# LiuZhu-CV/PAIF

Hardware: AMD Instinct MI355X
Metric: fused image-pairs/sec at 480x640 bs=8 per GPU (fusion-net forward) (higher is better)
Workload: dtype f16 (IEEE fp16 maps and conv weights, one fp16 MFMA per product, f32 accumulate; stems, guided filter and the last map fp32)

## Files before the change

paif_amd/csrc/conv_dma.hip:

```cpp
#include <stdint.h>
#include <stdlib.h>

#include <type_traits>

#include "conv_dma.h"
#include "conv_rows.h"

namespace paif_conv_dma {
namespace {

using namespace paif_rows;
constexpr int TW = 32, TH = 8;
#ifndef CD_PF
#define CD_PF 4
#endif
#ifndef CD_ST_AUX
#define CD_ST_AUX 2
#endif
#ifndef CD_EPI_SWAP
#define CD_EPI_SWAP 1
#endif
#ifndef CD_EPI_LINES
#define CD_EPI_LINES 1
#endif
#ifndef CD_EXP
#define CD_EXP 0
#endif
constexpr int PARK_WAVE = 2 * 32 * 32 * 4;
template <int DIL>
struct Geo {
  static constexpr int TWH = TW + 2 * DIL, THH = TH + 2 * DIL;
  static constexpr int NPIX = TWH * THH;
  static constexpr int DPW = (NPIX * 4 + 255) / 256;
  static constexpr int SLOT = 4 * DPW * 1024;
  static constexpr int PF = DIL == 1 ? CD_PF : 3;
  static constexpr int NSLOT = PF + 1;
  static constexpr int ROWB = TWH * 64;
  static constexpr int PARK_OFF = NSLOT * SLOT;
  static constexpr int lds_bytes(bool parked) { return PARK_OFF + (parked ? 4 * PARK_WAVE : 0); }
  static_assert(lds_bytes(true) <= 160 * 1024, "ring + transposition buffers exceed LDS");
  static_assert(4 * DPW * 64 >= NPIX * 4, "DMA instructions do not cover the halo tile");
  static __device__ __forceinline__ int base_row(int w) { return DIL == 1 ? 2 * w : (w >> 1) * 4 + (w & 1); }
};
constexpr int NSTORE = 4;
constexpr int VMCAP = 63;

#define CD_VMWAIT(n) ROWS_VMWAIT((n) > VMCAP ? VMCAP : (n))

template <int NSRC, int NRES, int PF, int DPW>
struct Sched {
  static constexpr int RL = 4 * NRES;
  static constexpr int smod(int x) { return ((x % NSRC) + NSRC) % NSRC; }
  static constexpr int R_STAGE = smod(1 - PF);
  static constexpr int D = (R_STAGE + PF - 1 - NSRC) / NSRC;
  static constexpr int U = D + (R_STAGE == 0 ? 2 : 1);
  static_assert(PF >= 2 && D >= 0 && U <= 4, "prefetch distance out of the range the tile loop lists");
  static constexpr int n1 = DPW * (PF - 1);
};

template <int NSRC, int NRES, int F, bool CP = false, int DIL = 1, int IA = 0>
__global__ __launch_bounds__(256, 1) void conv3x3_h16_dma(Args a, int ntiles, int tilesX, int tilesY) {
  typedef Geo<DIL> G;
  constexpr int TWH = G::TWH, NPIX = G::NPIX, DPW = G::DPW, SLOT = G::SLOT, PF = G::PF, NSLOT = G::NSLOT, ROWB = G::ROWB, PARK_OFF = G::PARK_OFF;
  typedef Sched<NSRC, NRES, PF, DPW> SC;
  constexpr bool SW = CD_EPI_SWAP && !CP && !(NRES == 3 && (NSRC == 3 || DIL == 2));
  constexpr int U = SW ? (SC::U + 1) & ~1 : SC::U, D = SC::D;
  constexpr int NACC = SW ? 2 : 1;
  __shared__ __attribute__((aligned(16))) unsigned char smem[G::lds_bytes(!SW)];
  asm volatile("" ::"v"((unsigned)(uintptr_t)(__attribute__((address_space(3))) unsigned char*)smem) : "memory");

  const int tid = threadIdx.x, l = tid & 63;
  const int w = __builtin_amdgcn_readfirstlane(tid >> 6);
  const int p = l & 31, hh = l >> 5;
  const int wb = G::base_row(w);

  const int xcd = blockIdx.x & 7, wg = blockIdx.x >> 3, nwg = gridDim.x >> 3;
  const int tpx = (ntiles + 7) >> 3;
  const int t_beg = xcd * tpx, t_end = min(ntiles, t_beg + tpx);
  const int cnt = t_beg + wg < t_end ? (t_end - t_beg - wg + nwg - 1) / nwg : 0;
  if (cnt == 0) return;
  const int H = a.H, W = a.W;
  auto pack_tile = [&](int k) -> unsigned {
    const int pos = wg + min(k, cnt - 1) * nwg;
    int t = a.reverse ? t_end - 1 - pos : t_beg + pos;
    const int tx = t % tilesX;
    t /= tilesX;
    const int ty = t % tilesY;
    return ((unsigned)(t / tilesY) << 22) | ((unsigned)ty << 11) | (unsigned)tx;
  };
  const unsigned tab0 = pack_tile(l), tab1 = pack_tile(l + 64);
  auto tile_of = [&](int k, int& b, int& y0, int& x0) -> bool {
    const bool ok = k >= 0 && k < cnt;
    const int kk = ok ? k : 0;
    const unsigned lo = __builtin_amdgcn_readlane(tab0, kk & 63), hi = __builtin_amdgcn_readlane(tab1, kk & 63);
    const unsigned pk = kk < 64 ? lo : hi;
    b = pk >> 22; y0 = ((pk >> 11) & 2047) * TH; x0 = (pk & 2047) * TW;
    return ok;
  };

  const int map_bytes = a.B * H * W * 64;
  __amdgpu_buffer_rsrc_t rs_src[NSRC];
#pragma unroll
  for (int s = 0; s < NSRC; ++s) rs_src[s] = __builtin_amdgcn_make_buffer_rsrc(const_cast<void*>(a.src[s]), 0, map_bytes, RSRC_W3);
  __amdgpu_buffer_rsrc_t rs_res[NRES > 0 ? NRES : 1];
#pragma unroll
  for (int r = 0; r < NRES; ++r) rs_res[r] = __builtin_amdgcn_make_buffer_rsrc(const_cast<void*>(a.res[r]), 0, map_bytes, RSRC_W3);
  const int opitch = a.cout * 2;
  const __amdgpu_buffer_rsrc_t rs_out = __builtin_amdgcn_make_buffer_rsrc(a.out, 0, a.B * H * W * opitch, RSRC_W3);
  const __amdgpu_buffer_rsrc_t rs_null = __builtin_amdgcn_make_buffer_rsrc(a.out, 0, 0, RSRC_W3);
  const __amdgpu_buffer_rsrc_t rs_cp = __builtin_amdgcn_make_buffer_rsrc(CP ? (void*)a.cpool : a.out, 0, CP ? a.B * H * W * 16 - 8 : 0, RSRC_W3);

  u32x4 bw[NSRC][9][2];
  {
    const __amdgpu_buffer_rsrc_t rs_w = __builtin_amdgcn_make_buffer_rsrc(const_cast<void*>(a.wpk), 0, NSRC * 9 * 2 * 2 * 1024, RSRC_W3);
#pragma unroll
    for (int s = 0; s < NSRC; ++s)
#pragma unroll
      for (int tap = 0; tap < 9; ++tap)
#pragma unroll
        for (int ks = 0; ks < 2; ++ks)
          bw[s][tap][ks] = __builtin_amdgcn_raw_buffer_load_b128(rs_w, (unsigned)l * 16u, (((s * 9 + tap) * 2 + ks) * 2) * 1024, 0);
  }
  constexpr int NEC = SW ? 16 : 8;
  float esc[NEC], esh[NEC];
#pragma unroll
  for (int j = 0; j < NEC; ++j) {
    const int c = SW ? ROWS_ACC_CHANNEL(j, hh) : 8 * (l & 3) + j;
    esc[j] = ((a.scale && c < a.cout) ? a.scale[c] : 1.f) * a.alpha;
    esh[j] = ((a.shift && c < a.cout) ? a.shift[c] : 0.f) * a.alpha;
  }
  const float e_slope = a.act == 1 ? *a.prelu : (a.act == 2 ? 0.f : 1.f);

  int d_rel[DPW];
  int d_rc[DPW];
#pragma unroll
  for (int i = 0; i < DPW; ++i) {
    const int n = (w * DPW + i) * 64 + l;
    const int pi = n >> 2;
    const int r = pi / TWH, c = pi - r * TWH;
    d_rel[i] = (r * W + c) * 64 + (((n & 3) ^ ((c >> 2) & 3)) * 16);
    d_rc[i] = pi < NPIX ? (r | (c << 8)) : -1;
  }
  unsigned d_voff[DPW];
  auto target = [&](int k) {
    int b, y0, x0;
    const bool ok = tile_of(k, b, y0, x0);
    const int org = ((b * H + y0 - DIL) * W + x0 - DIL) * 64;
#pragma unroll
    for (int i = 0; i < DPW; ++i) {
      const int gy = y0 - DIL + (d_rc[i] & 0xff), gx = x0 - DIL + (d_rc[i] >> 8);
      const bool in = !(CD_EXP & 4) && ok && d_rc[i] >= 0 && (unsigned)gy < (unsigned)H && (unsigned)gx < (unsigned)W;
      d_voff[i] = in ? (unsigned)(org + d_rel[i]) : OOB;
    }
  };
  unsigned a_rd[3][2];
#pragma unroll
  for (int dx = 0; dx < 3; ++dx)
#pragma unroll
    for (int ks = 0; ks < 2; ++ks) {
      const int c = p + dx * DIL;
      a_rd[dx][ks] = (unsigned)(wb * ROWB + c * 64 + (((2 * ks + hh) ^ ((c >> 2) & 3)) * 16));
    }
  const unsigned a_pw = PARK_OFF + w * PARK_WAVE + (4 * hh * 32 + p) * 4;
  const unsigned a_pr = PARK_OFF + w * PARK_WAVE + (l >> 2) * 128 + (l & 3) * 32;
  const unsigned e_lane = (unsigned)l * 16u;
  const unsigned o_lane = 8 * (l & 3) < a.cout ? (unsigned)((l >> 2) * opitch + (l & 3) * 16) : OOB;
  const unsigned e_lane_sw = (unsigned)(p * 64 + hh * 16);
  const unsigned o_lane_sw = (unsigned)(p * opitch + hh * 16);
  const unsigned o_lane_ln = ((l >> 4) & 1) * 16 < a.cout ? (unsigned)((l & 15) * opitch + ((l >> 4) & 1) * 32 + (l >> 5) * 16) : OOB;

  u32x4 rr[U][NRES > 0 ? NRES : 1][4];
  auto issue_res = [&](auto settag, int k) {
    constexpr int SET = decltype(settag)::value;
    int b, y0, x0;
    const bool ok = tile_of(k, b, y0, x0);
#pragma unroll
    for (int it = 0; it < 4; ++it) {
      const int y = y0 + wb + (it >> 1) * DIL, x = SW ? x0 + p : x0 + (it & 1) * 16 + (l >> 2);
      const bool in = ok && y < H && x < W;
      const unsigned soff = SW ? (unsigned)(((b * H + y) * W + x0) * 64 + (it & 1) * 32) : (unsigned)(((b * H + y) * W + x0 + (it & 1) * 16) * 64);
      const unsigned voff = in ? (SW ? e_lane_sw : e_lane) : OOB;
#pragma unroll
      for (int r = 0; r < NRES; ++r) rr[SET][r][it] = __builtin_amdgcn_raw_buffer_load_b128(rs_res[r], voff, soff, 0);
    }
  };

  auto relu_frag = [](u32x4& f) {
    typedef short s16x8 __attribute__((ext_vector_type(8)));
    const s16x8 z = {0, 0, 0, 0, 0, 0, 0, 0};
    f = __builtin_bit_cast(u32x4, __builtin_elementwise_max(__builtin_bit_cast(s16x8, f), z));
  };
  f32x16 acc[NACC][2];
  if constexpr (SW) {
#pragma unroll
    for (int r = 0; r < 16; ++r) acc[1][0][r] = acc[1][1][r] = 0.f;
  }
  u32x4 t[4][2];
#pragma unroll
  for (int it = 0; it < 4; ++it) t[it][0] = t[it][1] = u32x4{0, 0, 0, 0};
  float ev[8];
  u32x4 oq[2];
  float pmx = 0.f, psm = 0.f;
  int cur = NSLOT - PF;

  auto epi_park = [&](auto mtag, auto settag, bool pok, int pb, int py0, int px0) {
    constexpr int M = decltype(mtag)::value, SETP = decltype(settag)::value;
    constexpr int it = M / 9, j = M % 9;
    if constexpr (j < 8) {
      const unsigned raw = j < 4 ? t[it][0][j & 3] : t[it][1][j & 3];
      float v = __builtin_fmaf(__uint_as_float(raw), esc[j], esh[j]);
      v = __builtin_fmaf(e_slope, fminf(v, 0.f), fmaxf(v, 0.f));
#pragma unroll
      for (int r = 0; r < NRES; ++r) {
        const unsigned u = rr[SETP][r][it][j >> 1];
        if constexpr (F == 2) v += (float)__builtin_bit_cast(paif::f16x2_t, u)[j & 1];
        else v += __uint_as_float((j & 1) ? (u & 0xffff0000u) : (u << 16));
      }
      ev[j] = v;
      if constexpr (CP) {
        pmx = j == 0 ? v : fmaxf(pmx, v);
        psm = j == 0 ? v : psm + v;
      }
    } else {
      const uint2 o0 = paif::f32_to_h4<F>(make_float4(ev[0], ev[1], ev[2], ev[3]));
      const uint2 o1 = paif::f32_to_h4<F>(make_float4(ev[4], ev[5], ev[6], ev[7]));
      const int y = py0 + wb + (it >> 1) * DIL, x = px0 + (it & 1) * 16 + (l >> 2);
      const unsigned soff = (unsigned)(((pb * H + y) * W + px0 + (it & 1) * 16) * opitch);
      u32x4 od = {o0.x, o0.y, o1.x, o1.y};
      __builtin_amdgcn_raw_buffer_store_b128(od, rs_out, (!(CD_EXP & 1) && pok && y < H && x < W) ? o_lane : OOB, soff, CD_ST_AUX);
      asm volatile("s_nop 2" : "+v"(od));
      if constexpr (CP) {
        float mx = pmx, sm = psm;
        mx = fmaxf(mx, paif::dpp_f<0xB1>(mx)); sm += paif::dpp_f<0xB1>(sm);
        mx = fmaxf(mx, paif::dpp_f<0x4E>(mx)); sm += paif::dpp_f<0x4E>(sm);
        typedef float f32x2v __attribute__((ext_vector_type(2)));
        const f32x2v pv = {mx, sm * (1.0f / 32.0f)};
        const unsigned poff = (unsigned)(((pb * H + y) * W + px0 + (it & 1) * 16) * 16);
        __builtin_amdgcn_raw_buffer_store_b64(__builtin_bit_cast(unsigned __attribute__((ext_vector_type(2))), pv), rs_cp,
                                              (pok && y < H && x < W && (l & 3) == 0) ? (unsigned)((l >> 2) * 16) : OOB, poff, 0);
      }
    }
  };
  auto epi_swap = [&](auto mtag, auto settag, auto aptag, bool pok, int pb, int py0, int px0) {
    constexpr int M = decltype(mtag)::value, SETP = decltype(settag)::value, AP = decltype(aptag)::value;
    constexpr int row = M / 18, q = M % 18;
    if constexpr (q < 16) {
      constexpr int it = 2 * row + (q >> 3), j = q & 7;
      if constexpr (j == 0) {
#pragma unroll
        for (int r = 0; r < NRES; ++r) rr[SETP][r][it] = swap_unpack(rr[SETP][r][it]);
      }
      float v = __builtin_fmaf(acc[AP][row][q], esc[q], esh[q]);
      v = __builtin_fmaf(e_slope, fminf(v, 0.f), fmaxf(v, 0.f));
#pragma unroll
      for (int r = 0; r < NRES; ++r) {
        const unsigned u = rr[SETP][r][it][j >> 1];
        if constexpr (F == 2) v += (float)__builtin_bit_cast(paif::f16x2_t, u)[j & 1];
        else v += __uint_as_float((j & 1) ? (u & 0xffff0000u) : (u << 16));
      }
      if constexpr ((j & 1) == 0) ev[0] = v;
      else oq[q >> 3][j >> 1] = f32_to_h2<F>(ev[0], v);
    } else if constexpr (q == 16) {
      oq[0] = swap_unpack(oq[0]);
      oq[1] = swap_unpack(oq[1]);
      if constexpr (CD_EPI_LINES) line_swap(oq[0], oq[1]);
    } else {
      const int y = py0 + wb + row * DIL;
      const unsigned soff = (unsigned)(((pb * H + y) * W + px0) * opitch);
      const bool ok = !(CD_EXP & 1) && pok && y < H;
      if constexpr (CD_EPI_LINES) {
        const int x = px0 + (l & 15);
        __builtin_amdgcn_raw_buffer_store_b128(oq[0], rs_out, (ok && x < W) ? o_lane_ln : OOB, soff, CD_ST_AUX);
        __builtin_amdgcn_raw_buffer_store_b128(oq[1], rs_out, (ok && x + 16 < W) ? o_lane_ln : OOB, soff + (unsigned)(16 * opitch), CD_ST_AUX);
      } else {
        const int x = px0 + p;
        __builtin_amdgcn_raw_buffer_store_b128(oq[0], rs_out, (ok && x < W) ? o_lane_sw : OOB, soff, CD_ST_AUX);
        __builtin_amdgcn_raw_buffer_store_b128(oq[1], rs_out, (ok && x < W && a.cout > 16) ? o_lane_sw + 32u : OOB, soff, CD_ST_AUX);
      }
      asm volatile("s_nop 2" : "+v"(oq[0]), "+v"(oq[1]));
    }
  };
  auto epi = [&](auto mtag, auto settag, auto aptag, bool pok, int pb, int py0, int px0) {
    if constexpr (SW) epi_swap(mtag, settag, aptag, pok, pb, py0, px0);
    else epi_park(mtag, settag, pok, pb, py0, px0);
  };

  auto stage = [&](auto ktag, auto stag, auto virt, int k) {
    constexpr int K = decltype(ktag)::value, S = decltype(stag)::value;
    constexpr bool VIRT = decltype(virt)::value;
    constexpr int SETP = (K + U - 1) % U;
    constexpr int AC = SW ? K & 1 : 0, AP = SW ? AC ^ 1 : 0;
    const unsigned sb = (unsigned)cur * SLOT;
    const int fill = cur == 0 ? NSLOT - 1 : cur - 1;
    u32x4 A[2][4];
    unsigned ad[3][2];
    if constexpr (!VIRT) {
      CD_VMWAIT(SC::n1);
      asm volatile("s_barrier" ::: "memory");
#pragma unroll
      for (int dx = 0; dx < 3; ++dx)
#pragma unroll
        for (int ks = 0; ks < 2; ++ks) ad[dx][ks] = a_rd[dx][ks] + sb;
      if constexpr (S == 0 && !SW) {
#pragma unroll
        for (int it = 0; it < 4; ++it) {
          ROWS_RD128(t[it][0], a_pr, it * 2048);
          ROWS_RD128(t[it][1], a_pr, it * 2048 + 16);
        }
      }
#pragma unroll
      for (int r = 0; r < 4; ++r) ROWS_RD128(A[0][r], ad[0][0], r * DIL * ROWB);
    }
    if constexpr (NRES > 0 && S == SC::R_STAGE) issue_res(std::integral_constant<int, (K + D) % U>{}, k + D);
    asm volatile("" ::: "memory");
    if constexpr ((S + PF) % NSRC == 0) target(k + (S + PF) / NSRC);
#pragma unroll
    for (int i = 0; i < DPW; ++i) dma16<0>(rs_src[(S + PF) % NSRC], d_voff[i], (unsigned)(fill * SLOT + (w * DPW + i) * 1024));
    if constexpr (VIRT) {
      if constexpr (S == 0) {
#pragma unroll
        for (int it = 0; it < NSTORE; ++it) __builtin_amdgcn_raw_buffer_store_b128(u32x4{0, 0, 0, 0}, rs_null, 0, 0, 0);
      }
    } else {
      int pb = 0, py0 = 0, px0 = 0;
      bool pok = false;
      if constexpr (S == 0) pok = tile_of(k - 1, pb, py0, px0);
      auto mma = [&](auto gitag, auto dytag, auto jtag) {
        constexpr int gi = decltype(gitag)::value, dy = decltype(dytag)::value, j = decltype(jtag)::value;
        constexpr int ks = gi / 3, dx = gi % 3;
        if constexpr (!((CD_EXP & 2) && (dy > 0 || j > 0))) {
          const u32x4 pv = A[gi & 1][j + dy], wv = bw[S][dy * 3 + dx][ks];
          const u32x4 av = SW ? wv : pv, bv = SW ? pv : wv;
          if constexpr (S == 0 && gi == 0 && dy == 0) {
            const f32x16 z = {0.f, 0.f, 0.f, 0.f, 0.f, 0.f, 0.f, 0.f, 0.f, 0.f, 0.f, 0.f, 0.f, 0.f, 0.f, 0.f};
            acc[AC][j] = paif::mfma16<F>(av, bv, z);
          } else {
            acc[AC][j] = paif::mfma16<F>(av, bv, acc[AC][j]);
          }
        }
        if constexpr (S == 0)
          epi(std::integral_constant<int, gi * 6 + dy * 2 + j>{}, std::integral_constant<int, SETP>{}, std::integral_constant<int, AP>{}, pok, pb, py0, px0);
        if constexpr (IA == 2) {
          constexpr int call = dy * 2 + j;
          if constexpr (call == 0) relu_frag(A[gi & 1][1]);
          if constexpr (call == 2) relu_frag(A[gi & 1][2]);
          if constexpr (call == 4) relu_frag(A[gi & 1][3]);
        }
        __builtin_amdgcn_sched_barrier(0);
      };
      auto group = [&](auto gitag) {
        constexpr int gi = decltype(gitag)::value;
        if constexpr (gi + 1 < 6) {
          constexpr int ks1 = (gi + 1) / 3, dx1 = (gi + 1) % 3;
#pragma unroll
          for (int r = 0; r < 4; ++r) ROWS_RD128(A[(gi + 1) & 1][r], ad[dx1][ks1], r * DIL * ROWB);
        }
        if constexpr (S == 0 && gi == 0 && !SW) {
          asm volatile("s_waitcnt lgkmcnt(4)"
                       : "+v"(A[0][0]), "+v"(A[0][1]), "+v"(A[0][2]), "+v"(A[0][3]), "+v"(t[0][0]), "+v"(t[0][1]), "+v"(t[1][0]), "+v"(t[1][1]),
                         "+v"(t[2][0]), "+v"(t[2][1]), "+v"(t[3][0]), "+v"(t[3][1])::"memory");
        } else if constexpr (gi + 1 < 6) {
          asm volatile("s_waitcnt lgkmcnt(4)" : "+v"(A[gi & 1][0]), "+v"(A[gi & 1][1]), "+v"(A[gi & 1][2]), "+v"(A[gi & 1][3])::"memory");
        } else {
          asm volatile("s_waitcnt lgkmcnt(0)" : "+v"(A[gi & 1][0]), "+v"(A[gi & 1][1]), "+v"(A[gi & 1][2]), "+v"(A[gi & 1][3])::"memory");
        }
        if constexpr (IA == 2) relu_frag(A[gi & 1][0]);
        __builtin_amdgcn_sched_barrier(0);
        typedef std::integral_constant<int, 0> I0;
        typedef std::integral_constant<int, 1> I1;
        typedef std::integral_constant<int, 2> I2;
        mma(gitag, I0{}, I0{}); mma(gitag, I0{}, I1{});
        mma(gitag, I1{}, I0{}); mma(gitag, I1{}, I1{});
        mma(gitag, I2{}, I0{}); mma(gitag, I2{}, I1{});
      };
      group(std::integral_constant<int, 0>{});
      group(std::integral_constant<int, 1>{});
      group(std::integral_constant<int, 2>{});
      group(std::integral_constant<int, 3>{});
      group(std::integral_constant<int, 4>{});
      group(std::integral_constant<int, 5>{});
      if constexpr (S == NSRC - 1 && !SW) {
        asm volatile("s_nop 15\n\ts_nop 7" ::: "memory");
#pragma unroll
        for (int j = 0; j < 2; ++j)
#pragma unroll
          for (int r = 0; r < 16; ++r) {
            const float v = acc[0][j][r];
            ROWS_WR32(a_pw, v, (j * 32 + (r & 3) + 8 * (r >> 2)) * 128);
          }
      }
    }
    cur = cur == NSLOT - 1 ? 0 : cur + 1;
  };
  auto drain = [&](auto ktag, int k) {
    constexpr int K = decltype(ktag)::value;
    if constexpr (!SW) {
#pragma unroll
      for (int it = 0; it < 4; ++it) {
        ROWS_RD128(t[it][0], a_pr, it * 2048);
        ROWS_RD128(t[it][1], a_pr, it * 2048 + 16);
      }
      asm volatile("s_waitcnt lgkmcnt(0)"
                   : "+v"(t[0][0]), "+v"(t[0][1]), "+v"(t[1][0]), "+v"(t[1][1]), "+v"(t[2][0]), "+v"(t[2][1]), "+v"(t[3][0]), "+v"(t[3][1])::"memory");
    }
    int pb, py0, px0;
    const bool pok = tile_of(k, pb, py0, px0);
#define CD_M(m) epi(std::integral_constant<int, m>{}, std::integral_constant<int, K>{}, std::integral_constant<int, (SW ? K & 1 : 0)>{}, pok, pb, py0, px0);
    CD_M(0) CD_M(1) CD_M(2) CD_M(3) CD_M(4) CD_M(5) CD_M(6) CD_M(7) CD_M(8) CD_M(9) CD_M(10) CD_M(11)
    CD_M(12) CD_M(13) CD_M(14) CD_M(15) CD_M(16) CD_M(17) CD_M(18) CD_M(19) CD_M(20) CD_M(21) CD_M(22) CD_M(23)
    CD_M(24) CD_M(25) CD_M(26) CD_M(27) CD_M(28) CD_M(29) CD_M(30) CD_M(31) CD_M(32) CD_M(33) CD_M(34) CD_M(35)
#undef CD_M
  };

  auto vstage = [&](auto jtag) {
    constexpr int J = decltype(jtag)::value;
    constexpr int T = (J - (NSRC - 1)) / NSRC;
    constexpr int S = J - T * NSRC;
    constexpr int K = ((T % U) + U) % U;
    stage(std::integral_constant<int, K>{}, std::integral_constant<int, S>{}, std::true_type{}, T);
  };
  static_assert(PF >= 1 && PF <= 4, "the prologue lists up to 4 virtual stages");
  if constexpr (PF >= 4) vstage(std::integral_constant<int, -4>{});
  if constexpr (PF >= 3) vstage(std::integral_constant<int, -3>{});
  if constexpr (PF >= 2) vstage(std::integral_constant<int, -2>{});
  vstage(std::integral_constant<int, -1>{});

  auto tile_step = [&](auto ktag, int k) {
    stage(ktag, std::integral_constant<int, 0>{}, std::false_type{}, k);
    if constexpr (NSRC > 1) stage(ktag, std::integral_constant<int, 1>{}, std::false_type{}, k);
    if constexpr (NSRC > 2) stage(ktag, std::integral_constant<int, 2>{}, std::false_type{}, k);
  };
  static_assert(U <= 4, "the tile loop lists up to 4 tiles");
#define CD_TILE(i)                                                                                 \
  if constexpr (U > i) {                                                                           \
    tile_step(std::integral_constant<int, i % U>{}, k + i);                                        \
    if (k + i + 1 >= cnt) { drain(std::integral_constant<int, i % U>{}, k + i); break; }           \
  }
  for (int k = 0;; k += U) {
    CD_TILE(0) CD_TILE(1) CD_TILE(2) CD_TILE(3)
  }
#undef CD_TILE
  CD_VMWAIT(0);
}

namespace k7 {
constexpr int P = 3;
constexpr int TWH = TW + 2 * P, THH = TH + 2 * P;
constexpr int NPIX = TWH * THH;
constexpr int DPW = 9;
constexpr int SLOT = 4 * DPW * 1024;
constexpr int NSLOT = 2;
constexpr int ROWB = TWH * 64;
constexpr int WB_OFF = NSLOT * SLOT;
constexpr int WB_BYTES = 49 * 1024;
constexpr int PARK_OFF = WB_OFF + WB_BYTES;
constexpr bool SW = CD_EPI_SWAP;
constexpr int LDS_BYTES = PARK_OFF + (SW ? 0 : 4 * PARK_WAVE);
static_assert(LDS_BYTES <= 160 * 1024, "7x7: ring + weights + transposition buffers exceed LDS");
static_assert(4 * DPW * 64 >= NPIX * 4, "7x7: DMA instructions do not cover the halo tile");
}

template <int F>
__global__ __launch_bounds__(256, 1) void conv7x7_h16_dma(Args a, int ntiles, int tilesX, int tilesY) {
  constexpr int P = k7::P, TWH = k7::TWH, NPIX = k7::NPIX, DPW = k7::DPW, SLOT = k7::SLOT, ROWB = k7::ROWB, WB_OFF = k7::WB_OFF,
                PARK_OFF = k7::PARK_OFF;
  constexpr bool SW = k7::SW;
  constexpr int NACC = SW ? 2 : 1;
  __shared__ __attribute__((aligned(16))) unsigned char smem[k7::LDS_BYTES];
  asm volatile("" ::"v"((unsigned)(uintptr_t)(__attribute__((address_space(3))) unsigned char*)smem) : "memory");

  const int tid = threadIdx.x, l = tid & 63;
  const int w = __builtin_amdgcn_readfirstlane(tid >> 6);
  const int p = l & 31, hh = l >> 5;
  const int xcd = blockIdx.x & 7, wg = blockIdx.x >> 3, nwg = gridDim.x >> 3;
  const int tpx = (ntiles + 7) >> 3;
  const int t_beg = xcd * tpx, t_end = min(ntiles, t_beg + tpx);
  const int cnt = t_beg + wg < t_end ? (t_end - t_beg - wg + nwg - 1) / nwg : 0;
  if (cnt == 0) return;
  const int H = a.H, W = a.W;
  auto pack_tile = [&](int k) -> unsigned {
    const int pos = wg + min(k, cnt - 1) * nwg;
    int t = a.reverse ? t_end - 1 - pos : t_beg + pos;
    const int tx = t % tilesX;
    t /= tilesX;
    const int ty = t % tilesY;
    return ((unsigned)(t / tilesY) << 22) | ((unsigned)ty << 11) | (unsigned)tx;
  };
  const unsigned tab0 = pack_tile(l), tab1 = pack_tile(l + 64);
  auto tile_of = [&](int k, int& b, int& y0, int& x0) -> bool {
    const bool ok = k >= 0 && k < cnt;
    const int kk = ok ? k : 0;
    const unsigned lo = __builtin_amdgcn_readlane(tab0, kk & 63), hi = __builtin_amdgcn_readlane(tab1, kk & 63);
    const unsigned pk = kk < 64 ? lo : hi;
    b = pk >> 22; y0 = ((pk >> 11) & 2047) * TH; x0 = (pk & 2047) * TW;
    return ok;
  };
  const int map_bytes = a.B * H * W * 64;
  const __amdgpu_buffer_rsrc_t rs_src = __builtin_amdgcn_make_buffer_rsrc(const_cast<void*>(a.src[0]), 0, map_bytes, RSRC_W3);
  const __amdgpu_buffer_rsrc_t rs_out = __builtin_amdgcn_make_buffer_rsrc(a.out, 0, map_bytes, RSRC_W3);
  const __amdgpu_buffer_rsrc_t rs_w = __builtin_amdgcn_make_buffer_rsrc(const_cast<void*>(a.wpk), 0, 49 * 2 * 2 * 1024, RSRC_W3);

  u32x4 bw0[49];
#pragma unroll
  for (int tap = 0; tap < 49; ++tap) bw0[tap] = __builtin_amdgcn_raw_buffer_load_b128(rs_w, (unsigned)l * 16u, ((tap * 2 + 0) * 2) * 1024, 0);
#pragma unroll 1
  for (int i = tid; i < 49 * 64; i += 256) {
    const int tap = i >> 6, ln = i & 63;
    const u32x4 v = __builtin_amdgcn_raw_buffer_load_b128(rs_w, (unsigned)ln * 16u, ((tap * 2 + 1) * 2) * 1024, 0);
    const unsigned dst = WB_OFF + (unsigned)i * 16u;
    ROWS_WR128(dst, v, 0);
  }
  constexpr int NEC = SW ? 16 : 8;
  float esc[NEC], esh[NEC];
#pragma unroll
  for (int j = 0; j < NEC; ++j) {
    const int c = SW ? ROWS_ACC_CHANNEL(j, hh) : 8 * (l & 3) + j;
    esc[j] = (a.scale ? a.scale[c] : 1.f) * a.alpha;
    esh[j] = (a.shift ? a.shift[c] : 0.f) * a.alpha;
  }
  const float e_slope = a.act == 1 ? *a.prelu : (a.act == 2 ? 0.f : 1.f);

  int d_rel[DPW], d_rc[DPW];
#pragma unroll
  for (int i = 0; i < DPW; ++i) {
    const int n = (w * DPW + i) * 64 + l;
    const int pi = n >> 2;
    const int r = pi / TWH, c = pi - r * TWH;
    d_rel[i] = (r * W + c) * 64 + (((n & 3) ^ ((c >> 2) & 3)) * 16);
    d_rc[i] = pi < NPIX ? (r | (c << 8)) : -1;
  }
  unsigned d_voff[DPW];
  auto target = [&](int k) {
    int b, y0, x0;
    const bool ok = tile_of(k, b, y0, x0);
    const int org = ((b * H + y0 - P) * W + x0 - P) * 64;
#pragma unroll
    for (int i = 0; i < DPW; ++i) {
      const int gy = y0 - P + (d_rc[i] & 0xff), gx = x0 - P + (d_rc[i] >> 8);
      const bool in = ok && d_rc[i] >= 0 && (unsigned)gy < (unsigned)H && (unsigned)gx < (unsigned)W;
      d_voff[i] = in ? (unsigned)(org + d_rel[i]) : OOB;
    }
  };
  unsigned a_rd[7][2];
#pragma unroll
  for (int dx = 0; dx < 7; ++dx)
#pragma unroll
    for (int ks = 0; ks < 2; ++ks) {
      const int c = p + dx;
      a_rd[dx][ks] = (unsigned)(2 * w * ROWB + c * 64 + (((2 * ks + hh) ^ ((c >> 2) & 3)) * 16));
    }
  const unsigned a_wb = WB_OFF + (unsigned)l * 16u;
  const unsigned a_pw = PARK_OFF + w * PARK_WAVE + (4 * hh * 32 + p) * 4;
  const unsigned a_pr = PARK_OFF + w * PARK_WAVE + (l >> 2) * 128 + (l & 3) * 32;
  const unsigned e_lane = (unsigned)l * 16u;
  const unsigned e_lane_sw = (unsigned)(p * 64 + hh * 16);
  const unsigned e_lane_ln = (unsigned)((l & 15) * 64 + ((l >> 4) & 1) * 32 + (l >> 5) * 16);

  f32x16 acc[NACC][2];
  if constexpr (SW) {
#pragma unroll
    for (int r = 0; r < 16; ++r) acc[1][0][r] = acc[1][1][r] = 0.f;
  }
  u32x4 t[4][2];
#pragma unroll
  for (int it = 0; it < 4; ++it) t[it][0] = t[it][1] = u32x4{0, 0, 0, 0};
  float ev[8];
  u32x4 oq[2];
  auto epi = [&](auto mtag, auto aptag, bool pok, int pb, int py0, int px0) {
    constexpr int M = decltype(mtag)::value, AP = decltype(aptag)::value;
    if constexpr (SW) {
      constexpr int row = M / 18, q = M % 18;
      if constexpr (q < 16) {
        float v = __builtin_fmaf(acc[AP][row][q], esc[q], esh[q]);
        v = __builtin_fmaf(e_slope, fminf(v, 0.f), fmaxf(v, 0.f));
        if constexpr ((q & 1) == 0) ev[0] = v;
        else oq[q >> 3][(q & 7) >> 1] = f32_to_h2<F>(ev[0], v);
      } else if constexpr (q == 16) {
        oq[0] = swap_unpack(oq[0]);
        oq[1] = swap_unpack(oq[1]);
        if constexpr (CD_EPI_LINES) line_swap(oq[0], oq[1]);
      } else {
        const int y = py0 + 2 * w + row;
        const unsigned soff = (unsigned)(((pb * H + y) * W + px0) * 64);
        const bool ok = pok && y < H;
        if constexpr (CD_EPI_LINES) {
          const int x = px0 + (l & 15);
          __builtin_amdgcn_raw_buffer_store_b128(oq[0], rs_out, (ok && x < W) ? e_lane_ln : OOB, soff, CD_ST_AUX);
          __builtin_amdgcn_raw_buffer_store_b128(oq[1], rs_out, (ok && x + 16 < W) ? e_lane_ln : OOB, soff + 1024u, CD_ST_AUX);
        } else {
          const int x = px0 + p;
          __builtin_amdgcn_raw_buffer_store_b128(oq[0], rs_out, (ok && x < W) ? e_lane_sw : OOB, soff, CD_ST_AUX);
          __builtin_amdgcn_raw_buffer_store_b128(oq[1], rs_out, (ok && x < W) ? e_lane_sw + 32u : OOB, soff, CD_ST_AUX);
        }
        asm volatile("s_nop 2" : "+v"(oq[0]), "+v"(oq[1]));
      }
      return;
    }
    constexpr int it = M / 9, j = M % 9;
    if constexpr (j < 8) {
      const unsigned raw = j < 4 ? t[it][0][j & 3] : t[it][1][j & 3];
      float v = __builtin_fmaf(__uint_as_float(raw), esc[j], esh[j]);
      ev[j] = __builtin_fmaf(e_slope, fminf(v, 0.f), fmaxf(v, 0.f));
    } else {
      const uint2 o0 = paif::f32_to_h4<F>(make_float4(ev[0], ev[1], ev[2], ev[3]));
      const uint2 o1 = paif::f32_to_h4<F>(make_float4(ev[4], ev[5], ev[6], ev[7]));
      const int y = py0 + 2 * w + (it >> 1), x = px0 + (it & 1) * 16 + (l >> 2);
      const unsigned soff = (unsigned)(((pb * H + y) * W + px0 + (it & 1) * 16) * 64);
      u32x4 od = {o0.x, o0.y, o1.x, o1.y};
      __builtin_amdgcn_raw_buffer_store_b128(od, rs_out, (pok && y < H && x < W) ? e_lane : OOB, soff, CD_ST_AUX);
      asm volatile("s_nop 2" : "+v"(od));
    }
  };

  asm volatile("s_waitcnt lgkmcnt(0)" ::: "memory");
  target(0);
#pragma unroll
  for (int i = 0; i < DPW; ++i) dma16<0>(rs_src, d_voff[i], (unsigned)((w * DPW + i) * 1024));
  int cur = 0;
  auto tile = [&](auto actag, int k) {
    constexpr int AC = decltype(actag)::value, AP = SW ? AC ^ 1 : 0;
    const unsigned sb = (unsigned)cur * SLOT;
    CD_VMWAIT(0);
    asm volatile("s_barrier" ::: "memory");
    unsigned ad[7][2];
#pragma unroll
    for (int dx = 0; dx < 7; ++dx)
#pragma unroll
      for (int ks = 0; ks < 2; ++ks) ad[dx][ks] = a_rd[dx][ks] + sb;
    u32x4 A[2][8], BL[7];
    if constexpr (!SW) {
#pragma unroll
      for (int it = 0; it < 4; ++it) {
        ROWS_RD128(t[it][0], a_pr, it * 2048);
        ROWS_RD128(t[it][1], a_pr, it * 2048 + 16);
      }
    }
#pragma unroll
    for (int r = 0; r < 8; ++r) ROWS_RD128(A[0][r], ad[0][0], r * ROWB);
    target(k + 1);
#pragma unroll
    for (int i = 0; i < DPW; ++i) dma16<0>(rs_src, d_voff[i], (unsigned)((cur ^ 1) * SLOT + (w * DPW + i) * 1024));
    int pb, py0, px0;
    const bool pok = tile_of(k - 1, pb, py0, px0);
    auto mma = [&](auto gitag, auto dytag, auto jtag) {
      constexpr int gi = decltype(gitag)::value, dy = decltype(dytag)::value, j = decltype(jtag)::value;
      constexpr int dx = gi >> 1, ks = gi & 1;
      const u32x4 pv = A[gi & 1][j + dy];
      const u32x4 wv = ks == 0 ? bw0[dy * 7 + dx] : BL[dy];
      const u32x4 av = SW ? wv : pv, bv = SW ? pv : wv;
      if constexpr (gi == 0 && dy == 0) {
        const f32x16 z = {0.f, 0.f, 0.f, 0.f, 0.f, 0.f, 0.f, 0.f, 0.f, 0.f, 0.f, 0.f, 0.f, 0.f, 0.f, 0.f};
        acc[AC][j] = paif::mfma16<F>(av, bv, z);
      } else {
        acc[AC][j] = paif::mfma16<F>(av, bv, acc[AC][j]);
      }
      constexpr int m = gi * 14 + dy * 2 + j;
      if constexpr (m < 36) epi(std::integral_constant<int, m>{}, std::integral_constant<int, AP>{}, pok, pb, py0, px0);
      __builtin_amdgcn_sched_barrier(0);
    };
    auto group = [&](auto gitag) {
      constexpr int gi = decltype(gitag)::value;
      if constexpr (gi + 1 < 14) {
        constexpr int dx1 = (gi + 1) >> 1, ks1 = (gi + 1) & 1;
#pragma unroll
        for (int r = 0; r < 8; ++r) ROWS_RD128(A[(gi + 1) & 1][r], ad[dx1][ks1], r * ROWB);
        if constexpr (ks1 == 1) {
#pragma unroll
          for (int dy = 0; dy < 7; ++dy) ROWS_RD128(BL[dy], a_wb, (dy * 7 + dx1) * 1024);
        }
      }
      if constexpr (gi == 0 && !SW) {
        asm volatile("s_waitcnt lgkmcnt(15)"
                     : "+v"(A[0][0]), "+v"(A[0][1]), "+v"(A[0][2]), "+v"(A[0][3]), "+v"(A[0][4]), "+v"(A[0][5]), "+v"(A[0][6]), "+v"(A[0][7]),
                       "+v"(t[0][0]), "+v"(t[0][1]), "+v"(t[1][0]), "+v"(t[1][1]), "+v"(t[2][0]), "+v"(t[2][1]), "+v"(t[3][0])::"memory");
        asm volatile("" : "+v"(t[3][1])::"memory");
      } else if constexpr (gi + 1 >= 14) {
        asm volatile("s_waitcnt lgkmcnt(0)"
                     : "+v"(A[1][0]), "+v"(A[1][1]), "+v"(A[1][2]), "+v"(A[1][3]), "+v"(A[1][4]), "+v"(A[1][5]), "+v"(A[1][6]), "+v"(A[1][7]),
                       "+v"(BL[0]), "+v"(BL[1]), "+v"(BL[2]), "+v"(BL[3]), "+v"(BL[4]), "+v"(BL[5]), "+v"(BL[6])::"memory");
      } else if constexpr ((gi & 1) == 1) {
        asm volatile("s_waitcnt lgkmcnt(8)"
                     : "+v"(A[1][0]), "+v"(A[1][1]), "+v"(A[1][2]), "+v"(A[1][3]), "+v"(A[1][4]), "+v"(A[1][5]), "+v"(A[1][6]), "+v"(A[1][7]),
                       "+v"(BL[0]), "+v"(BL[1]), "+v"(BL[2]), "+v"(BL[3]), "+v"(BL[4]), "+v"(BL[5]), "+v"(BL[6])::"memory");
      } else {
        asm volatile("s_waitcnt lgkmcnt(15)"
                     : "+v"(A[0][0]), "+v"(A[0][1]), "+v"(A[0][2]), "+v"(A[0][3]), "+v"(A[0][4]), "+v"(A[0][5]), "+v"(A[0][6]), "+v"(A[0][7])::"memory");
      }
      __builtin_amdgcn_sched_barrier(0);
      typedef std::integral_constant<int, 0> J0;
      typedef std::integral_constant<int, 1> J1;
#define CD_DY(d) mma(gitag, std::integral_constant<int, d>{}, J0{}); mma(gitag, std::integral_constant<int, d>{}, J1{});
      CD_DY(0) CD_DY(1) CD_DY(2) CD_DY(3) CD_DY(4) CD_DY(5) CD_DY(6)
#undef CD_DY
    };
#define CD_G(g) group(std::integral_constant<int, g>{});
    CD_G(0) CD_G(1) CD_G(2) CD_G(3) CD_G(4) CD_G(5) CD_G(6) CD_G(7) CD_G(8) CD_G(9) CD_G(10) CD_G(11) CD_G(12) CD_G(13)
#undef CD_G
    if constexpr (!SW) {
      asm volatile("s_nop 15\n\ts_nop 7" ::: "memory");
#pragma unroll
      for (int j = 0; j < 2; ++j)
#pragma unroll
        for (int r = 0; r < 16; ++r) {
          const float v = acc[0][j][r];
          ROWS_WR32(a_pw, v, (j * 32 + (r & 3) + 8 * (r >> 2)) * 128);
        }
    }
    cur ^= 1;
  };
  auto drain = [&](auto aptag) {
    if constexpr (!SW) {
#pragma unroll
      for (int it = 0; it < 4; ++it) {
        ROWS_RD128(t[it][0], a_pr, it * 2048);
        ROWS_RD128(t[it][1], a_pr, it * 2048 + 16);
      }
      asm volatile("s_waitcnt lgkmcnt(0)"
                   : "+v"(t[0][0]), "+v"(t[0][1]), "+v"(t[1][0]), "+v"(t[1][1]), "+v"(t[2][0]), "+v"(t[2][1]), "+v"(t[3][0]), "+v"(t[3][1])::"memory");
    }
    int pb, py0, px0;
    const bool pok = tile_of(cnt - 1, pb, py0, px0);
#define CD_M(m) epi(std::integral_constant<int, m>{}, aptag, pok, pb, py0, px0);
    CD_M(0) CD_M(1) CD_M(2) CD_M(3) CD_M(4) CD_M(5) CD_M(6) CD_M(7) CD_M(8) CD_M(9) CD_M(10) CD_M(11)
    CD_M(12) CD_M(13) CD_M(14) CD_M(15) CD_M(16) CD_M(17) CD_M(18) CD_M(19) CD_M(20) CD_M(21) CD_M(22) CD_M(23)
    CD_M(24) CD_M(25) CD_M(26) CD_M(27) CD_M(28) CD_M(29) CD_M(30) CD_M(31) CD_M(32) CD_M(33) CD_M(34) CD_M(35)
#undef CD_M
  };
  typedef std::integral_constant<int, 0> T0;
  typedef std::integral_constant<int, 1> T1;
  if constexpr (SW) {
    for (int k = 0;; k += 2) {
      tile(T0{}, k);
      if (k + 1 >= cnt) { drain(T0{}); break; }
      tile(T1{}, k + 1);
      if (k + 2 >= cnt) { drain(T1{}); break; }
    }
  } else {
    for (int k = 0; k < cnt; ++k) tile(T0{}, k);
    drain(T0{});
  }
  CD_VMWAIT(0);
}

int launch_7(const Args& a, hipStream_t st) {
  const int tilesX = (a.W + TW - 1) / TW, tilesY = (a.H + TH - 1) / TH;
  if (a.f16) hipLaunchKernelGGL(conv7x7_h16_dma<2>, dim3(256), dim3(256), 0, st, a, a.B * tilesX * tilesY, tilesX, tilesY);
  else hipLaunchKernelGGL(conv7x7_h16_dma<1>, dim3(256), dim3(256), 0, st, a, a.B * tilesX * tilesY, tilesX, tilesY);
  hipError_t e = hipGetLastError();
  if (e != hipSuccess) {
    paif::set_error("conv2d(bf16 dma 7x7): launch failed: %s", hipGetErrorString(e));
    return (int)e;
  }
  return 0;
}

template <int NSRC, int NRES>
int launch_n(const Args& a, hipStream_t st) {
  const int tilesX = (a.W + TW - 1) / TW, tilesY = (a.H + TH - 1) / TH;
  if (a.cpool) {
    if constexpr (NSRC == 3 && (NRES == 1 || NRES == 3)) {
      if (a.f16) hipLaunchKernelGGL((conv3x3_h16_dma<NSRC, NRES, 2, true>), dim3(256), dim3(256), 0, st, a, a.B * tilesX * tilesY, tilesX, tilesY);
      else hipLaunchKernelGGL((conv3x3_h16_dma<NSRC, NRES, 1, true>), dim3(256), dim3(256), 0, st, a, a.B * tilesX * tilesY, tilesX, tilesY);
    } else {
      paif::set_error("conv2d(dma): the fused ChannelPool is built for 3 sources with 1 or 3 residual maps");
      return PAIF_ENOSUP;
    }
  } else if (a.f16) hipLaunchKernelGGL((conv3x3_h16_dma<NSRC, NRES, 2>), dim3(256), dim3(256), 0, st, a, a.B * tilesX * tilesY, tilesX, tilesY);
  else hipLaunchKernelGGL((conv3x3_h16_dma<NSRC, NRES, 1>), dim3(256), dim3(256), 0, st, a, a.B * tilesX * tilesY, tilesX, tilesY);
  hipError_t e = hipGetLastError();
  if (e != hipSuccess) {
    paif::set_error("conv2d(h16 dma): launch failed: %s", hipGetErrorString(e));
    return (int)e;
  }
  return 0;
}

template <int NRES, bool CP>
int launch_d2(const Args& a, hipStream_t st) {
  const int tilesX = (a.W + TW - 1) / TW, tilesY = (a.H + TH - 1) / TH;
  if (a.f16) hipLaunchKernelGGL((conv3x3_h16_dma<1, NRES, 2, CP, 2, 2>), dim3(256), dim3(256), 0, st, a, a.B * tilesX * tilesY, tilesX, tilesY);
  else hipLaunchKernelGGL((conv3x3_h16_dma<1, NRES, 1, CP, 2, 2>), dim3(256), dim3(256), 0, st, a, a.B * tilesX * tilesY, tilesX, tilesY);
  hipError_t e = hipGetLastError();
  if (e != hipSuccess) {
    paif::set_error("conv2d(h16 dma, dilation 2): launch failed: %s", hipGetErrorString(e));
    return (int)e;
  }
  return 0;
}

}

bool is_1x1(const Args& a);
int launch_1x1(const Args& a, hipStream_t st);
bool is_rows(const Args& a);
int launch_rows(const Args& a, hipStream_t st);

static bool is_tile(const Args& a) {
  static const bool on = [] {
    const char* e = getenv("PAIF_CONV_DMA");
    return !(e && e[0] == '0');
  }();
  static const bool on_d2 = [] {
    const char* e = getenv("PAIF_CONV_DMA_D2");
    return !(e && e[0] == '0');
  }();
  if (!on || a.out_f32 || !(a.alpha > 0.f)) return false;
  bool built;
  if (a.dil == 2)
    built = on_d2 && a.kh == 3 && a.cout == 32 && a.in_relu && a.nsrc == 1 && (a.nres == 1 || a.nres == 3);
  else if (a.in_relu || a.dil != 1)
    built = false;
  else if (a.kh == 3 && a.cout == 32)
    built = a.nsrc >= 1 && a.nsrc <= 3 && a.nres >= 0 && a.nres <= (a.nsrc == 1 ? 1 : 3);
  else
    built = ((a.kh == 3 && a.cout == 16) || (a.kh == 7 && a.cout == 32)) && a.nsrc == 1 && a.nres == 0;
  const long long tiles = (long long)a.B * ((a.H + TH - 1) / TH) * ((a.W + TW - 1) / TW);
  return built && tiles >= 1024 && tiles <= 128 * 256 && a.B < 1024 && a.H < 2048 * TH && a.W < 2048 * TW &&
         (long long)a.B * a.H * a.W * 64 < (1ll << 31);
}

Form classify(const Args& a) {
  if (is_1x1(a)) return ONE_BY_ONE;
  if (is_rows(a)) return ROWS;
  return is_tile(a) ? TILE : NONE;
}

bool can_cpool(const Args& a) {
  return a.kh == 3 && a.cout == 32 && (a.nres == 1 || a.nres == 3) && ((a.dil == 1 && a.nsrc == 3) || (a.dil == 2 && a.nsrc == 1));
}

int launch(const Args& a, hipStream_t st) {
  switch (classify(a)) {
    case ONE_BY_ONE: return launch_1x1(a, st);
    case ROWS: return launch_rows(a, st);
    case TILE: break;
    default:
      paif::set_error("conv2d(h16 dma): no LDS-DMA kernel is built for this descriptor and shape");
      return PAIF_ENOSUP;
  }
  if (a.cpool && !can_cpool(a)) {
    paif::set_error("conv2d(dma): no fused ChannelPool for this form");
    return PAIF_ENOSUP;
  }
  if (a.kh == 7) return launch_7(a, st);
  if (a.dil == 2) {
    if (a.nres == 1) return a.cpool ? launch_d2<1, true>(a, st) : launch_d2<1, false>(a, st);
    return a.cpool ? launch_d2<3, true>(a, st) : launch_d2<3, false>(a, st);
  }
  switch (a.nsrc * 10 + a.nres) {
    case 10: return launch_n<1, 0>(a, st);
    case 11: return launch_n<1, 1>(a, st);
    case 20: return launch_n<2, 0>(a, st);
    case 21: return launch_n<2, 1>(a, st);
    case 22: return launch_n<2, 2>(a, st);
    case 23: return launch_n<2, 3>(a, st);
    case 30: return launch_n<3, 0>(a, st);
    case 31: return launch_n<3, 1>(a, st);
    case 32: return launch_n<3, 2>(a, st);
    case 33: return launch_n<3, 3>(a, st);
    default: break;
  }
  paif::set_error("conv2d(bf16 dma): %d sources / %d residual maps not built", a.nsrc, a.nres);
  return PAIF_ENOSUP;
}

}
```

Before: 2687.

## Overlap stage head (wait, barrier, DMA issue, first A load) with MFMA groups

Adds a head-overlap mode, on by default for non-dilated, non-CP convs. It moves each stage's vmcnt wait, barrier, residual loads, DMA issues, next-slot address setup and target computation into gaps interleaved between the MFMA groups of the previous stage. The first A fragment of the next slot is preloaded at the end of the stage, and a prologue is added to prime it. The aim is to hide the per-stage head latency behind matrix math. In exchange it shortens the prefetch wait depth by one slot and makes the LDS wait-count bookkeeping more delicate.

```diff
diff --git a/paif_amd/csrc/conv_dma.hip b/paif_amd/csrc/conv_dma.hip
--- a/paif_amd/csrc/conv_dma.hip
+++ b/paif_amd/csrc/conv_dma.hip
@@ -22,6 +22,9 @@
 #endif
 #ifndef CD_EPI_LINES
 #define CD_EPI_LINES 1
+#endif
+#ifndef CD_HEAD_OVERLAP
+#define CD_HEAD_OVERLAP 1
 #endif
 #ifndef CD_EXP
 #define CD_EXP 0
@@ -56,7 +59,9 @@
   static constexpr int U = D + (R_STAGE == 0 ? 2 : 1);
   static_assert(PF >= 2 && D >= 0 && U <= 4, "prefetch distance out of the range the tile loop lists");
   static constexpr int n1 = DPW * (PF - 1);
+  static constexpr int n1_ho = DPW * (PF - 2);
 };
+constexpr bool head_overlap_form(int NSRC, int NRES, bool CP, int DIL) { return DIL == 1 && !CP; }
 
 template <int NSRC, int NRES, int F, bool CP = false, int DIL = 1, int IA = 0>
 __global__ __launch_bounds__(256, 1) void conv3x3_h16_dma(Args a, int ntiles, int tilesX, int tilesY) {
@@ -66,6 +71,7 @@
   constexpr bool SW = CD_EPI_SWAP && !CP && !(NRES == 3 && (NSRC == 3 || DIL == 2));
   constexpr int U = SW ? (SC::U + 1) & ~1 : SC::U, D = SC::D;
   constexpr int NACC = SW ? 2 : 1;
+  constexpr bool HO = CD_HEAD_OVERLAP && head_overlap_form(NSRC, NRES, CP, DIL);
   __shared__ __attribute__((aligned(16))) unsigned char smem[G::lds_bytes(!SW)];
   asm volatile("" ::"v"((unsigned)(uintptr_t)(__attribute__((address_space(3))) unsigned char*)smem) : "memory");
 
@@ -142,16 +148,22 @@
     d_rc[i] = pi < NPIX ? (r | (c << 8)) : -1;
   }
   unsigned d_voff[DPW];
+  int tg_y0 = 0, tg_x0 = 0, tg_org = 0;
+  bool tg_ok = false;
+  auto target_tile = [&](int k) {
+    int b;
+    tg_ok = tile_of(k, b, tg_y0, tg_x0);
+    tg_org = ((b * H + tg_y0 - DIL) * W + tg_x0 - DIL) * 64;
+  };
+  auto target_off = [&](int i) {
+    const int gy = tg_y0 - DIL + (d_rc[i] & 0xff), gx = tg_x0 - DIL + (d_rc[i] >> 8);
+    const bool in = !(CD_EXP & 4) && tg_ok && d_rc[i] >= 0 && (unsigned)gy < (unsigned)H && (unsigned)gx < (unsigned)W;
+    d_voff[i] = in ? (unsigned)(tg_org + d_rel[i]) : OOB;
+  };
   auto target = [&](int k) {
-    int b, y0, x0;
-    const bool ok = tile_of(k, b, y0, x0);
-    const int org = ((b * H + y0 - DIL) * W + x0 - DIL) * 64;
-#pragma unroll
-    for (int i = 0; i < DPW; ++i) {
-      const int gy = y0 - DIL + (d_rc[i] & 0xff), gx = x0 - DIL + (d_rc[i] >> 8);
-      const bool in = !(CD_EXP & 4) && ok && d_rc[i] >= 0 && (unsigned)gy < (unsigned)H && (unsigned)gx < (unsigned)W;
-      d_voff[i] = in ? (unsigned)(org + d_rel[i]) : OOB;
-    }
+    target_tile(k);
+#pragma unroll
+    for (int i = 0; i < DPW; ++i) target_off(i);
   };
   unsigned a_rd[3][2];
 #pragma unroll
@@ -170,12 +182,12 @@
   const unsigned o_lane_ln = ((l >> 4) & 1) * 16 < a.cout ? (unsigned)((l & 15) * opitch + ((l >> 4) & 1) * 32 + (l >> 5) * 16) : OOB;
 
   u32x4 rr[U][NRES > 0 ? NRES : 1][4];
-  auto issue_res = [&](auto settag, int k) {
-    constexpr int SET = decltype(settag)::value;
+  auto issue_res = [&](auto settag, int k, auto lotag, auto hitag) {
+    constexpr int SET = decltype(settag)::value, LO = decltype(lotag)::value, HI = decltype(hitag)::value;
     int b, y0, x0;
     const bool ok = tile_of(k, b, y0, x0);
 #pragma unroll
-    for (int it = 0; it < 4; ++it) {
+    for (int it = LO; it < HI; ++it) {
       const int y = y0 + wb + (it >> 1) * DIL, x = SW ? x0 + p : x0 + (it & 1) * 16 + (l >> 2);
       const bool in = ok && y < H && x < W;
       const unsigned soff = SW ? (unsigned)(((b * H + y) * W + x0) * 64 + (it & 1) * 32) : (unsigned)(((b * H + y) * W + x0 + (it & 1) * 16) * 64);
@@ -202,6 +214,8 @@
   u32x4 oq[2];
   float pmx = 0.f, psm = 0.f;
   int cur = NSLOT - PF;
+  u32x4 A[2][4];
+  unsigned ad[3][2];
 
   auto epi_park = [&](auto mtag, auto settag, bool pok, int pb, int py0, int px0) {
     constexpr int M = decltype(mtag)::value, SETP = decltype(settag)::value;
@@ -292,15 +306,8 @@
     constexpr int AC = SW ? K & 1 : 0, AP = SW ? AC ^ 1 : 0;
     const unsigned sb = (unsigned)cur * SLOT;
     const int fill = cur == 0 ? NSLOT - 1 : cur - 1;
-    u32x4 A[2][4];
-    unsigned ad[3][2];
-    if constexpr (!VIRT) {
-      CD_VMWAIT(SC::n1);
-      asm volatile("s_barrier" ::: "memory");
-#pragma unroll
-      for (int dx = 0; dx < 3; ++dx)
-#pragma unroll
-        for (int ks = 0; ks < 2; ++ks) ad[dx][ks] = a_rd[dx][ks] + sb;
+    const unsigned sbn = (unsigned)(cur == NSLOT - 1 ? 0 : cur + 1) * SLOT;
+    if constexpr (!VIRT && HO) {
       if constexpr (S == 0 && !SW) {
 #pragma unroll
         for (int it = 0; it < 4; ++it) {
@@ -308,14 +315,48 @@
           ROWS_RD128(t[it][1], a_pr, it * 2048 + 16);
         }
       }
+    }
+    if constexpr (!VIRT && !HO) {
+      CD_VMWAIT(SC::n1);
+      asm volatile("s_barrier" ::: "memory");
+#pragma unroll
+      for (int dx = 0; dx < 3; ++dx)
+#pragma unroll
+        for (int ks = 0; ks < 2; ++ks) ad[dx][ks] = a_rd[dx][ks] + sb;
+      if constexpr (S == 0 && !SW) {
+#pragma unroll
+        for (int it = 0; it < 4; ++it) {
+          ROWS_RD128(t[it][0], a_pr, it * 2048);
+          ROWS_RD128(t[it][1], a_pr, it * 2048 + 16);
+        }
+      }
 #pragma unroll
       for (int r = 0; r < 4; ++r) ROWS_RD128(A[0][r], ad[0][0], r * DIL * ROWB);
     }
-    if constexpr (NRES > 0 && S == SC::R_STAGE) issue_res(std::integral_constant<int, (K + D) % U>{}, k + D);
-    asm volatile("" ::: "memory");
-    if constexpr ((S + PF) % NSRC == 0) target(k + (S + PF) / NSRC);
-#pragma unroll
-    for (int i = 0; i < DPW; ++i) dma16<0>(rs_src[(S + PF) % NSRC], d_voff[i], (unsigned)(fill * SLOT + (w * DPW + i) * 1024));
+    typedef std::integral_constant<int, (K + D) % U> RSET;
+    if constexpr (VIRT || !HO) {
+      if constexpr (NRES > 0 && S == SC::R_STAGE) issue_res(RSET{}, k + D, std::integral_constant<int, 0>{}, std::integral_constant<int, 4>{});
+      asm volatile("" ::: "memory");
+      if constexpr ((S + PF) % NSRC == 0) target(k + (S + PF) / NSRC);
+#pragma unroll
+      for (int i = 0; i < DPW; ++i) dma16<0>(rs_src[(S + PF) % NSRC], d_voff[i], (unsigned)(fill * SLOT + (w * DPW + i) * 1024));
+    }
+    auto gap = [&](auto mtag) {
+      constexpr int M = decltype(mtag)::value;
+      if constexpr (M == 0) {
+        CD_VMWAIT(SC::n1_ho);
+        asm volatile("s_barrier" ::: "memory");
+      }
+      if constexpr (NRES > 0 && S == SC::R_STAGE && M < 2)
+        issue_res(RSET{}, k + D, std::integral_constant<int, 2 * M>{}, std::integral_constant<int, 2 * M + 2>{});
+      if constexpr (M >= 2 && M < 2 + DPW)
+        dma16<0>(rs_src[(S + PF) % NSRC], d_voff[M - 2], (unsigned)(fill * SLOT + (w * DPW + M - 2) * 1024));
+      if constexpr (M % 6 == 1) ad[(M / 6) % 3][M / 18] = a_rd[(M / 6) % 3][M / 18] + sbn;
+      if constexpr ((S + 1 + PF) % NSRC == 0) {
+        if constexpr (M == 18) target_tile(k + (S + 1 + PF) / NSRC);
+        if constexpr (M >= 19 && M < 19 + DPW) target_off(M - 19);
+      }
+    };
     if constexpr (VIRT) {
       if constexpr (S == 0) {
 #pragma unroll
@@ -338,6 +379,7 @@
             acc[AC][j] = paif::mfma16<F>(av, bv, acc[AC][j]);
           }
         }
+        if constexpr (HO) gap(std::integral_constant<int, gi * 6 + dy * 2 + j>{});
         if constexpr (S == 0)
           epi(std::integral_constant<int, gi * 6 + dy * 2 + j>{}, std::integral_constant<int, SETP>{}, std::integral_constant<int, AP>{}, pok, pb, py0, px0);
         if constexpr (IA == 2) {
@@ -354,8 +396,17 @@
           constexpr int ks1 = (gi + 1) / 3, dx1 = (gi + 1) % 3;
 #pragma unroll
           for (int r = 0; r < 4; ++r) ROWS_RD128(A[(gi + 1) & 1][r], ad[dx1][ks1], r * DIL * ROWB);
+        } else if constexpr (HO) {
+#pragma unroll
+          for (int r = 0; r < 4; ++r) ROWS_RD128(A[0][r], ad[0][0], r * DIL * ROWB);
         }
-        if constexpr (S == 0 && gi == 0 && !SW) {
+        if constexpr (HO && gi == 0) {
+          if constexpr (S == 0 && !SW)
+            asm volatile("s_waitcnt lgkmcnt(4)"
+                         : "+v"(t[0][0]), "+v"(t[0][1]), "+v"(t[1][0]), "+v"(t[1][1]), "+v"(t[2][0]), "+v"(t[2][1]), "+v"(t[3][0]), "+v"(t[3][1])::"memory");
+        } else if constexpr (HO && gi == 5) {
+          asm volatile("s_waitcnt lgkmcnt(4)" : "+v"(A[1][0]), "+v"(A[1][1]), "+v"(A[1][2]), "+v"(A[1][3])::"memory");
+        } else if constexpr (S == 0 && gi == 0 && !SW) {
           asm volatile("s_waitcnt lgkmcnt(4)"
                        : "+v"(A[0][0]), "+v"(A[0][1]), "+v"(A[0][2]), "+v"(A[0][3]), "+v"(t[0][0]), "+v"(t[0][1]), "+v"(t[1][0]), "+v"(t[1][1]),
                          "+v"(t[2][0]), "+v"(t[2][1]), "+v"(t[3][0]), "+v"(t[3][1])::"memory");
@@ -389,6 +440,7 @@
             ROWS_WR32(a_pw, v, (j * 32 + (r & 3) + 8 * (r >> 2)) * 128);
           }
       }
+      if constexpr (HO) asm volatile("s_waitcnt lgkmcnt(0)" : "+v"(A[0][0]), "+v"(A[0][1]), "+v"(A[0][2]), "+v"(A[0][3])::"memory");
     }
     cur = cur == NSLOT - 1 ? 0 : cur + 1;
   };
@@ -424,6 +476,18 @@
   if constexpr (PF >= 3) vstage(std::integral_constant<int, -3>{});
   if constexpr (PF >= 2) vstage(std::integral_constant<int, -2>{});
   vstage(std::integral_constant<int, -1>{});
+  if constexpr (HO) {
+    if constexpr (PF % NSRC == 0) target(PF / NSRC);
+    CD_VMWAIT(SC::n1);
+    asm volatile("s_barrier" ::: "memory");
+#pragma unroll
+    for (int dx = 0; dx < 3; ++dx)
+#pragma unroll
+      for (int ks = 0; ks < 2; ++ks) ad[dx][ks] = a_rd[dx][ks] + (unsigned)cur * SLOT;
+#pragma unroll
+    for (int r = 0; r < 4; ++r) ROWS_RD128(A[0][r], ad[0][0], r * DIL * ROWB);
+    asm volatile("s_waitcnt lgkmcnt(0)" : "+v"(A[0][0]), "+v"(A[0][1]), "+v"(A[0][2]), "+v"(A[0][3])::"memory");
+  }
 
   auto tile_step = [&](auto ktag, int k) {
     stage(ktag, std::integral_constant<int, 0>{}, std::false_type{}, k);
```

New measurement: 2702 (median of 6 runs). Within noise of the previous version (+0.5%).
